# dingwentao/GPU-lossless-compression

Hardware: AMD Instinct MI355X
Metric: encode+decode GB/s (input bytes) per GPU and whole-node; compression ratio parity (higher is better)
Workload: dtype u8; 1 GPU; configs[1]: 4 GiB/GPU Zipf(1.0) bytes (Philox4x32-10, key 0x5eed0002, counter = byte index / 4), 1 MiB blocks, cudppCompress BWT+MTF+Huffman encode; block_bytes=1048576, blocks_per_gpu=4096, batch_rows=2048, batch_rows_asked=2048, output_layout=compact, drain_between_steps=False, parallelism=blocks round-robin over 1 GPU(s), no data-path collective, blocks_left_by_bucket_sorter=0, blocks_left_by_sample_sorter=0

## Files before the change

### gpu-lossless-compression_amd/csrc/mtf.hip

```cpp
#include "glc_device.h"
#include "glc_internal.h"

namespace glc {

constexpr int MTF_WAVES = 4;
constexpr int MTF_INP = 256 + 8;

__global__ __launch_bounds__(MTF_WAVES * 64) void k_mtf_chunk_lists(const uint8_t *__restrict__ in,
                                                                   size_t in_stride, uint32_t n,
                                                                   uint8_t *__restrict__ lists,
                                                                   uint16_t *__restrict__ lens,
                                                                   uint32_t max_chunks, const uint32_t *__restrict__ only)
{
    __shared__ uint32_t s_first[MTF_WAVES][256];
    __shared__ unsigned long long s_bm[MTF_WAVES][64];
    __shared__ uint32_t s_cum[MTF_WAVES][64];
    const uint32_t b = blockIdx.y, l = threadIdx.x & 63;
    if (only && !only[b]) return;
    const uint32_t w = __builtin_amdgcn_readfirstlane(threadIdx.x >> 6);
    const uint32_t chunk = blockIdx.x * MTF_WAVES + w;
    const uint32_t nchunks = (n + MTF_CHUNK - 1) / MTF_CHUNK;
    if (chunk >= nchunks) return;
    const uint32_t lo = chunk * MTF_CHUNK, hi = min(n, lo + MTF_CHUNK), C = hi - lo;
    const uint8_t *src = in + (size_t)b * in_stride;
    uint8_t *L = lists + ((size_t)b * max_chunks + chunk) * 256;
    uint32_t *first = s_first[w];
    for (int i = l; i < 256; i += 64) first[i] = 0xFFFFFFFFu;
    s_bm[w][l] = 0;
    __builtin_amdgcn_wave_barrier();
    if (C == MTF_CHUNK && (reinterpret_cast<uintptr_t>(src + lo) & 15) == 0) {
        uint4 q[4];
#pragma unroll
        for (int g = 0; g < 4; g++)
            q[g] = *reinterpret_cast<const uint4 *>(src + lo + MTF_CHUNK - 1024 * g - 16 * (l + 1));
#pragma unroll
        for (int g = 0; g < 4; g++) {
            const uint32_t d[4] = {q[g].x, q[g].y, q[g].z, q[g].w};
#pragma unroll
            for (int k = 15; k >= 0; k--) {
                const uint32_t sym = (d[k >> 2] >> (8 * (k & 3))) & 0xFFu, o = 1024u * g + 16u * l + 15u - k;
                if (o < first[sym]) atomicMin(&first[sym], o);
            }
        }
    } else {
        for (uint32_t o = l; o < C; o += 64) {
            const uint32_t sym = src[hi - 1 - o];
            if (o < first[sym]) atomicMin(&first[sym], o);
        }
    }
    __builtin_amdgcn_wave_barrier();
    uint32_t f[4];
#pragma unroll
    for (int j = 0; j < 4; j++) {
        f[j] = first[4 * l + j];
        if (f[j] != 0xFFFFFFFFu) atomicOr(&s_bm[w][f[j] >> 6], 1ull << (f[j] & 63));
    }
    __builtin_amdgcn_wave_barrier();
    const uint32_t c = (uint32_t)__popcll(s_bm[w][l]);
    const uint32_t inc = wave_incl_add(c);
    s_cum[w][l] = inc - c;
    __builtin_amdgcn_wave_barrier();
#pragma unroll
    for (int j = 0; j < 4; j++) {
        if (f[j] != 0xFFFFFFFFu) {
            const uint32_t wd = f[j] >> 6, r = f[j] & 63;
            L[s_cum[w][wd] + (uint32_t)__popcll(s_bm[w][wd] & ((1ull << r) - 1ull))] = (uint8_t)(4 * l + j);
        }
    }
    if (l == 0) lens[(size_t)b * max_chunks + chunk] = (uint16_t)__builtin_amdgcn_readlane((int)inc, 63);
}



__device__ __forceinline__ uint32_t mtf_fold(const uint8_t *cur, uint8_t *next, uint8_t *inp, uint32_t p4, uint32_t m,
                                             uint32_t ls, uint32_t l, uint32_t *cur4 = nullptr)
{
    const uint32_t c4 = reinterpret_cast<const uint32_t *>(cur)[l];
    reinterpret_cast<uint32_t *>(inp)[l] = 0;
    __builtin_amdgcn_wave_barrier();
    reinterpret_cast<uint32_t *>(next)[l] = p4;
#pragma unroll
    for (int j = 0; j < 4; j++) inp[4 * l + j < m ? (p4 >> (8 * j)) & 0xFFu : 256u + j] = 1;
    __builtin_amdgcn_wave_barrier();
    if (cur4) *cur4 = c4;
    uint32_t in[4];
#pragma unroll
    for (int j = 0; j < 4; j++) in[j] = inp[(c4 >> (8 * j)) & 0xFFu];
    uint32_t keep[4], cnt = 0;
#pragma unroll
    for (int j = 0; j < 4; j++) { keep[j] = (4 * l + j < ls && !in[j]) ? 1u : 0u; cnt += keep[j]; }
    const uint32_t inc = wave_incl_add(cnt);
    uint32_t pos = m + inc - cnt;
#pragma unroll
    for (int j = 0; j < 4; j++) {
        if (keep[j]) next[pos] = (uint8_t)(c4 >> (8 * j));
        pos += keep[j];
    }
    __builtin_amdgcn_wave_barrier();
    return m + (uint32_t)__builtin_amdgcn_readlane((int)inc, 63);
}

template <int MSC_WAVES>
__global__ __launch_bounds__(MSC_WAVES * 64) void k_mtf_scan_lists(uint8_t *__restrict__ lists,
                                                                  const uint16_t *__restrict__ lens, uint32_t n,
                                                                  uint32_t max_chunks, const uint32_t *__restrict__ only)
{
    constexpr int MSC_GROUP = 256 / MSC_WAVES;
    __shared__ __attribute__((aligned(16))) uint8_t s_state[MSC_WAVES][2][256];
    __shared__ __attribute__((aligned(16))) uint8_t s_inp[MSC_WAVES][MTF_INP];
    __shared__ __attribute__((aligned(16))) uint8_t s_comb[MSC_WAVES][256];
    __shared__ uint32_t s_clen[MSC_WAVES];
    __shared__ __attribute__((aligned(16))) uint8_t s_start[MSC_WAVES + 1][256];
    __shared__ __attribute__((aligned(16))) uint8_t s_carry[256];
    const uint32_t b = blockIdx.x, l = threadIdx.x & 63;
    if (only && !only[b]) return;
    const uint32_t w = __builtin_amdgcn_readfirstlane(threadIdx.x >> 6);
    const uint32_t nchunks = (n + MTF_CHUNK - 1) / MTF_CHUNK;
    uint8_t *LB = lists + (size_t)b * max_chunks * 256;
    const uint16_t *NB = lens + (size_t)b * max_chunks;
    if (w == 0) for (int i = l; i < 256; i += 64) s_carry[i] = (uint8_t)i;
    for (uint32_t r0 = 0; r0 < nchunks; r0 += MSC_WAVES * MSC_GROUP) {
        const uint32_t nch = min(nchunks - r0, (uint32_t)(MSC_WAVES * MSC_GROUP));
        const uint32_t ngroups = (nch + MSC_GROUP - 1) / MSC_GROUP;
        const uint32_t c0 = r0 + w * MSC_GROUP, c1 = min(r0 + nch, c0 + MSC_GROUP);
        uint32_t p4[MSC_GROUP], mm[MSC_GROUP];
#pragma unroll
        for (int k = 0; k < MSC_GROUP; k++) {
            const bool in = c0 + k < c1;
            p4[k] = in ? reinterpret_cast<const uint32_t *>(LB + (size_t)(c0 + k) * 256)[l] : 0u;
            mm[k] = in ? NB[c0 + k] : 0u;
        }
        if (w < ngroups) {
            int cur = 0;
            uint32_t ls = 0;
#pragma unroll
            for (int k = 0; k < MSC_GROUP; k++)
                if (c0 + k < c1) { ls = mtf_fold(s_state[w][cur], s_state[w][cur ^ 1], s_inp[w], p4[k], mm[k], ls, l); cur ^= 1; }
            reinterpret_cast<uint32_t *>(s_comb[w])[l] = reinterpret_cast<const uint32_t *>(s_state[w][cur])[l];
            if (l == 0) s_clen[w] = ls;
        }
        __syncthreads();
        if (w == 0) {
            reinterpret_cast<uint32_t *>(s_start[0])[l] = reinterpret_cast<const uint32_t *>(s_carry)[l];
            uint32_t cp[MSC_WAVES], cl[MSC_WAVES];
#pragma unroll
            for (int g = 0; g < MSC_WAVES; g++) { cp[g] = reinterpret_cast<const uint32_t *>(s_comb[g])[l]; cl[g] = s_clen[g]; }
            __builtin_amdgcn_wave_barrier();
#pragma unroll
            for (int g = 0; g < MSC_WAVES; g++)
                if ((uint32_t)g < ngroups) (void)mtf_fold(s_start[g], s_start[g + 1], s_inp[0], cp[g], cl[g], 256, l);
            reinterpret_cast<uint32_t *>(s_carry)[l] = reinterpret_cast<const uint32_t *>(s_start[ngroups])[l];
        }
        __syncthreads();
        if (w < ngroups) {
            int cur = 0;
            reinterpret_cast<uint32_t *>(s_state[w][0])[l] = reinterpret_cast<const uint32_t *>(s_start[w])[l];
            __builtin_amdgcn_wave_barrier();
#pragma unroll
            for (int k = 0; k < MSC_GROUP; k++) {
                if (c0 + k < c1) {
                    uint32_t st4;
                    if (c0 + k + 1 < c1) { (void)mtf_fold(s_state[w][cur], s_state[w][cur ^ 1], s_inp[w], p4[k], mm[k], 256, l, &st4); cur ^= 1; }
                    else st4 = reinterpret_cast<const uint32_t *>(s_state[w][cur])[l];
                    reinterpret_cast<uint32_t *>(LB + (size_t)(c0 + k) * 256)[l] = st4;
                }
            }
        }
        __syncthreads();
    }
}

constexpr int MTF_ROWS = 4;
constexpr int MTF_NWORDS = 32;
constexpr uint32_t MTF_SEG = 1024;
#ifndef GLC_MTF_QUARTERS_MAX
#define GLC_MTF_QUARTERS_MAX 2048
#endif
constexpr uint32_t MTF_QUARTERS_MAX_CHUNKS = GLC_MTF_QUARTERS_MAX;

__device__ __forceinline__ void mtf_rebase(uint32_t *tab, unsigned long long *bm, uint16_t *cum, uint32_t lr)
{
#pragma unroll 4
    for (int k = 0; k < 16; k++) {
        const uint32_t c = 16u * (uint32_t)k + lr;
        const uint32_t t = tab[c] >> 16, wd = t >> 6;
        const uint32_t kb = cum[wd] + (uint32_t)__popcll(bm[wd] << (63u - (t & 63u)));
        tab[c] = (t - kb) << 16;
    }
    __builtin_amdgcn_wave_barrier();
    bm[2 * lr] = 0; bm[2 * lr + 1] = 0;
    reinterpret_cast<uint32_t *>(cum)[lr] = 0;
    __builtin_amdgcn_wave_barrier();
}

__device__ __forceinline__ uint32_t mtf_slide(uint32_t Pb)
{
    uint32_t G = 0, t0;
#define GLC_SLIDE(K)                                                                                    \
    "v_sub_co_u32_dpp %1, vcc, %2, %2 row_shr:" #K " row_mask:0xf bank_mask:0xf bound_ctrl:1\n\t"            \
    "v_addc_co_u32_e32 %0, vcc, 0, %0, vcc\n\t"
    asm volatile(GLC_SLIDE(1) GLC_SLIDE(2) GLC_SLIDE(3) GLC_SLIDE(4) GLC_SLIDE(5) GLC_SLIDE(6) GLC_SLIDE(7) GLC_SLIDE(8)
                 GLC_SLIDE(9) GLC_SLIDE(10) GLC_SLIDE(11) GLC_SLIDE(12) GLC_SLIDE(13) GLC_SLIDE(14) GLC_SLIDE(15)
                 : "+v"(G), "=&v"(t0) : "v"(Pb) : "vcc");
#undef GLC_SLIDE
    return G;
}

__device__ __forceinline__ void mtf_recount(const unsigned long long *bm, uint16_t *cum, uint32_t lr)
{
    const uint4 v = *reinterpret_cast<const uint4 *>(bm + 2 * lr);
    const uint32_t c0 = (uint32_t)__builtin_popcount(v.x) + (uint32_t)__builtin_popcount(v.y);
    const uint32_t sum = c0 + (uint32_t)__builtin_popcount(v.z) + (uint32_t)__builtin_popcount(v.w);
    uint32_t inc = sum;
    inc += GLC_DPP(inc, 0x111, 0xf);
    inc += GLC_DPP(inc, 0x112, 0xf);
    inc += GLC_DPP(inc, 0x114, 0xf);
    inc += GLC_DPP(inc, 0x118, 0xf);
    const uint32_t r0 = inc - sum;
    reinterpret_cast<uint32_t *>(cum)[lr] = r0 | ((r0 + c0) << 16);
}


#ifndef GLC_MTF_REQ_DIST
#define GLC_MTF_REQ_DIST 1
#endif
constexpr int MTF_REQ = GLC_MTF_REQ_DIST;
#ifndef GLC_MTF_FULL_GROUP
#define GLC_MTF_FULL_GROUP 4
#endif
constexpr int MTF_GROUP = GLC_MTF_FULL_GROUP;
static_assert(MTF_REQ >= 1 && MTF_GROUP % MTF_REQ == 0 && MTF_SEG % (16 * MTF_GROUP) == 0 && MTF_CHUNK % MTF_SEG == 0, "group shape");

template <bool WITH_HIST, bool ZEROS, bool LASTG>
__device__ __forceinline__ void mtf_full_group(const uint8_t *__restrict__ sb, uint8_t *__restrict__ db, uint32_t voff,
                                               uint32_t lbg, uint32_t (&q)[MTF_REQ], uint32_t *tab, unsigned long long *bm,
                                               uint16_t *cum, uint32_t *hist, uint32_t lr, uint32_t row)
{
    const uint32_t mybit = 1u << lr, below = mybit - 1u;
    const uint8_t *sp = sb + voff;
    uint8_t *dp = db + voff;
    uint16_t *killp = reinterpret_cast<uint16_t *>(bm) + ((lbg + 256u) >> 4);
#pragma unroll
    for (int j = 0; j < MTF_GROUP; j++) {
        const uint32_t lb = lbg + 16u * j;
        const uint32_t sym = q[0];
#pragma unroll
        for (int d = 0; d + 1 < MTF_REQ; d++) q[d] = q[d + 1];
        if (!LASTG || j + MTF_REQ < MTF_GROUP) q[MTF_REQ - 1] = sp[16 * (j + MTF_REQ)];
        atomicOr(&tab[sym], mybit);
        __builtin_amdgcn_wave_barrier();
        const uint32_t e = tab[sym];
        const uint32_t before = e & below;
        const bool hasprev = before != 0;
        const uint32_t p = 31u - (uint32_t)__builtin_clz(before | 1u);
        const bool last_in_batch = ((e & 0xFFFFu) >> lr) == 1u;
        uint32_t Pb = hasprev ? lb + p + 257u : (e >> 16) + 1u;
        asm volatile("s_nop 1" : "+v"(Pb));
        const uint32_t T = mtf_slide(Pb) + lr - 15u;
        const uint32_t bitx = Pb - 1u;
        uint32_t o;
        if (hasprev) o = T - (p + 1u);
        else {
            const uint32_t wd = bitx >> 6, r = bitx & 63;
            const uint32_t kb = cum[wd] + (uint32_t)__popcll(bm[wd] << (63u - r));
            o = T + kb + 255u - bitx;
        }
        __builtin_amdgcn_wave_barrier();
        {
            const uint64_t nl = __ballot(!last_in_batch);
            if (lr == 0) killp[j] = (uint16_t)(nl >> (16u * row));
        }
        if (WITH_HIST && ZEROS) {
            const uint64_t zb = __ballot(o == 0);
            const uint32_t zrow = (uint32_t)(zb >> (16u * row)) & 0xFFFFu;
            if (lr == 0 && zrow) atomicAdd(&hist[0], (uint32_t)__builtin_popcount(zrow));
        }
        dp[16 * j] = (uint8_t)o;
        if (WITH_HIST && !(ZEROS && o == 0)) atomicAdd(&hist[o & 127], 1u << ((o >> 3) & 16));
        if (!hasprev) atomicOr(&reinterpret_cast<uint32_t *>(bm)[bitx >> 5], 1u << (bitx & 31));
        if (last_in_batch) tab[sym] = (lb + lr + 256u) << 16;
        __builtin_amdgcn_wave_barrier();
        mtf_recount(bm, cum, lr);
        __builtin_amdgcn_wave_barrier();
    }
}

template <bool WITH_HIST, bool ZEROS>
__device__ __forceinline__ void mtf_encode_full_row(const uint8_t *__restrict__ sb, uint8_t *__restrict__ db, uint32_t lo,
                                                    const uint8_t *__restrict__ list, uint32_t *tab, unsigned long long *bm,
                                                    uint16_t *cum, uint32_t *hist, uint32_t *__restrict__ H, uint32_t lr,
                                                    uint32_t row)
{
    {
        const uint4 lw = reinterpret_cast<const uint4 *>(list)[lr];
        const uint32_t q[4] = {lw.x, lw.y, lw.z, lw.w};
#pragma unroll
        for (int j = 0; j < 16; j++) tab[(q[j >> 2] >> (8 * (j & 3))) & 0xFF] = (255u - (16 * lr + j)) << 16;
        bm[2 * lr] = 0; bm[2 * lr + 1] = 0;
        reinterpret_cast<uint32_t *>(cum)[lr] = 0;
        if (WITH_HIST) for (int i = lr; i < 128; i += 16) hist[i] = 0;
        __builtin_amdgcn_wave_barrier();
    }
    uint32_t voff = lo + lr;
    uint32_t q[MTF_REQ];
#pragma unroll
    for (int d = 0; d < MTF_REQ; d++) q[d] = sb[voff + 16u * d];
    constexpr uint32_t NSEG = MTF_CHUNK / MTF_SEG, NGRP = MTF_SEG / (16 * MTF_GROUP);
    for (uint32_t seg = 0; seg < NSEG; seg++) {
        if (seg) mtf_rebase(tab, bm, cum, lr);
        const uint32_t ng = seg + 1 < NSEG ? NGRP : NGRP - 1;
        for (uint32_t g = 0; g < ng; g++, voff += 16 * MTF_GROUP)
            mtf_full_group<WITH_HIST, ZEROS, false>(sb, db, voff, 16 * MTF_GROUP * g, q, tab, bm, cum, hist, lr, row);
    }
    mtf_full_group<WITH_HIST, ZEROS, true>(sb, db, voff, 16 * MTF_GROUP * (NGRP - 1), q, tab, bm, cum, hist, lr, row);
    if (WITH_HIST) {
        __builtin_amdgcn_wave_barrier();
        if constexpr (SUBHIST_PACKED) for (int i = lr; i < 128; i += 16) H[i] = hist[i];
        else for (int i = lr; i < 256; i += 16) H[i] = (hist[i & 127] >> (16 * (i >> 7))) & 0xFFFFu;
    }
}

template <bool WITH_HIST, bool QUARTERS, bool ZEROS = false, bool FULL = false>
__global__ __launch_bounds__(MTF_WAVES * 64) void k_mtf_encode(const uint8_t *__restrict__ in,
                                                              size_t in_stride, uint32_t n,
                                                              const uint8_t *__restrict__ lists,
                                                              uint32_t max_chunks,
                                                              uint8_t *__restrict__ out, size_t out_stride,
                                                              uint32_t *__restrict__ sub_hist, const uint32_t *__restrict__ only)
{
    __shared__ uint32_t s_hist[WITH_HIST ? MTF_WAVES * MTF_ROWS : 1][128 + 8];
    __shared__ uint32_t s_tab[MTF_WAVES * MTF_ROWS][256 + 8];
    __shared__ __attribute__((aligned(16))) unsigned long long s_bm[MTF_WAVES * MTF_ROWS][MTF_NWORDS + 2];
    __shared__ __attribute__((aligned(16))) uint16_t s_cum[MTF_WAVES * MTF_ROWS][MTF_NWORDS + 8];
    __shared__ __attribute__((aligned(16))) uint8_t s_qstart[QUARTERS ? MTF_WAVES : 1][MTF_ROWS][256];
    __shared__ __attribute__((aligned(16))) uint8_t s_qlist[QUARTERS ? MTF_WAVES : 1][256], s_qinp[QUARTERS ? MTF_WAVES : 1][MTF_INP];
    __shared__ uint32_t s_qfirst[QUARTERS ? MTF_WAVES : 1][256], s_qcum[QUARTERS ? MTF_WAVES : 1][16];
    __shared__ unsigned long long s_qbm[QUARTERS ? MTF_WAVES : 1][16];
    const uint32_t b = blockIdx.y, l = threadIdx.x & 63, lr = l & 15, row = l >> 4;
    if (only && !only[b]) return;
    const uint32_t w = threadIdx.x >> 6, slot = w * MTF_ROWS + row;
    const uint32_t nchunks = (n + MTF_CHUNK - 1) / MTF_CHUNK;
    constexpr uint32_t QLEN = MTF_CHUNK / MTF_ROWS;
    const uint32_t chunk0 = QUARTERS ? blockIdx.x * MTF_WAVES + w : (blockIdx.x * MTF_WAVES + w) * MTF_ROWS;
    if (chunk0 >= nchunks) return;
    const uint32_t chunk = QUARTERS ? chunk0 : chunk0 + row;
    if constexpr (FULL) {
        static_assert(!QUARTERS, "the rows of the FULL form are whole chunks");
        mtf_encode_full_row<WITH_HIST, ZEROS>(in + (size_t)b * in_stride, out + (size_t)b * out_stride, chunk * MTF_CHUNK,
                                              lists + ((size_t)b * max_chunks + chunk) * 256, s_tab[slot], s_bm[slot], s_cum[slot],
                                              s_hist[WITH_HIST ? slot : 0], sub_hist + ((size_t)b * max_chunks + chunk) * SUBHIST_DWORDS, lr, row);
        return;
    }
    const uint32_t Cc0 = min(n, chunk0 * MTF_CHUNK + MTF_CHUNK) - chunk0 * MTF_CHUNK;
    bool live;
    uint32_t lo, C, Cmax;
    if (QUARTERS) {
        live = Cc0 > QLEN * row;
        lo = chunk0 * MTF_CHUNK + (live ? QLEN * row : 0u);
        C = live ? min(Cc0 - QLEN * row, QLEN) : 0u;
        Cmax = min(Cc0, QLEN);
    } else {
        live = chunk < nchunks;
        lo = (live ? chunk : chunk0) * MTF_CHUNK;
        C = live ? min(n, lo + MTF_CHUNK) - lo : 0u;
        Cmax = Cc0;
    }
    const uint8_t *src = in + (size_t)b * in_stride + lo;
    uint8_t *dst = out + (size_t)b * out_stride + lo;
    uint32_t *tab = s_tab[slot];
    unsigned long long *bm = s_bm[slot];
    uint16_t *cum = s_cum[slot];
    uint4 lw;
    if (QUARTERS) {
        uint8_t (*S)[256] = s_qstart[w];
        reinterpret_cast<uint32_t *>(S[0])[l] = reinterpret_cast<const uint32_t *>(lists + ((size_t)b * max_chunks + chunk0) * 256)[l];
        const uint8_t *cbase = in + (size_t)b * in_stride + chunk0 * MTF_CHUNK;
        const bool vec = (reinterpret_cast<uintptr_t>(cbase) & 15) == 0;
        for (uint32_t q = 0; q + 1 < MTF_ROWS && Cc0 > QLEN * (q + 1); q++) {
            uint32_t *first = s_qfirst[w];
            for (int i = l; i < 256; i += 64) first[i] = 0xFFFFFFFFu;
            if (l < 16) s_qbm[w][l] = 0;
            __builtin_amdgcn_wave_barrier();
            const uint8_t *qs = cbase + QLEN * q;
            if (vec) {
                const uint4 v = *reinterpret_cast<const uint4 *>(qs + QLEN - 16 * (l + 1));
                const uint32_t d[4] = {v.x, v.y, v.z, v.w};
#pragma unroll
                for (int k = 15; k >= 0; k--) {
                    const uint32_t sym = (d[k >> 2] >> (8 * (k & 3))) & 0xFFu, o = 16u * l + 15u - k;
                    if (o < first[sym]) atomicMin(&first[sym], o);
                }
            } else {
                for (uint32_t o = l; o < QLEN; o += 64) {
                    const uint32_t sym = qs[QLEN - 1 - o];
                    if (o < first[sym]) atomicMin(&first[sym], o);
                }
            }
            __builtin_amdgcn_wave_barrier();
            uint32_t f[4];
#pragma unroll
            for (int j = 0; j < 4; j++) {
                f[j] = first[4 * l + j];
                if (f[j] != 0xFFFFFFFFu) atomicOr(&s_qbm[w][f[j] >> 6], 1ull << (f[j] & 63));
            }
            __builtin_amdgcn_wave_barrier();
            const uint32_t c = l < 16 ? (uint32_t)__popcll(s_qbm[w][l]) : 0u;
            const uint32_t inc = wave_incl_add(c);
            if (l < 16) s_qcum[w][l] = inc - c;
            __builtin_amdgcn_wave_barrier();
            uint8_t *L = s_qlist[w];
#pragma unroll
            for (int j = 0; j < 4; j++) {
                if (f[j] != 0xFFFFFFFFu) {
                    const uint32_t wd = f[j] >> 6, r = f[j] & 63;
                    L[s_qcum[w][wd] + (uint32_t)__popcll(s_qbm[w][wd] & ((1ull << r) - 1ull))] = (uint8_t)(4 * l + j);
                }
            }
            __builtin_amdgcn_wave_barrier();
            const uint32_t m = (uint32_t)__builtin_amdgcn_readlane((int)inc, 63);
            (void)mtf_fold(S[q], S[q + 1], s_qinp[w], reinterpret_cast<const uint32_t *>(L)[l], m, 256, l);
        }
        __builtin_amdgcn_wave_barrier();
        lw = reinterpret_cast<const uint4 *>(S[live ? row : 0])[lr];
    } else {
        lw = reinterpret_cast<const uint4 *>(lists + ((size_t)b * max_chunks + (live ? chunk : chunk0)) * 256)[lr];
    }
    {
        const uint32_t q[4] = {lw.x, lw.y, lw.z, lw.w};
#pragma unroll
        for (int j = 0; j < 16; j++) tab[(q[j >> 2] >> (8 * (j & 3))) & 0xFF] = (255u - (16 * lr + j)) << 16;
        bm[2 * lr] = 0; bm[2 * lr + 1] = 0;
        reinterpret_cast<uint32_t *>(cum)[lr] = 0;
        if (WITH_HIST) for (int i = lr; i < 128; i += 16) s_hist[slot][i] = 0;
        __builtin_amdgcn_wave_barrier();
    }
    const uint32_t mybit = 1u << lr, below = mybit - 1u;
    uint32_t sym_next = src[lr < C ? lr : 0u];
    for (uint32_t seg0 = 0; seg0 < Cmax; seg0 += MTF_SEG) {
        if (seg0) {
#pragma unroll 4
            for (int k = 0; k < 16; k++) {
                const uint32_t c = 16u * (uint32_t)k + lr;
                const uint32_t t = tab[c] >> 16, wd = t >> 6;
                const uint32_t kb = cum[wd] + (uint32_t)__popcll(bm[wd] << (63u - (t & 63u)));
                tab[c] = (t - kb) << 16;
            }
            __builtin_amdgcn_wave_barrier();
            bm[2 * lr] = 0; bm[2 * lr + 1] = 0;
            reinterpret_cast<uint32_t *>(cum)[lr] = 0;
            __builtin_amdgcn_wave_barrier();
        }
        const uint32_t seg_end = min(Cmax, seg0 + MTF_SEG);
        for (uint32_t base = seg0; base < seg_end; base += 16) {
            const uint32_t i = base + lr, lb = base - seg0;
            const bool valid = i < C;
            const uint32_t sym = sym_next;
            sym_next = src[i + 16 < C ? i + 16 : 0u];
            if (valid) atomicOr(&tab[sym], mybit);
            __builtin_amdgcn_wave_barrier();
            const uint32_t e = tab[sym];
            const uint32_t before = e & below;
            const bool hasprev = before != 0;
            const uint32_t p = 31u - (uint32_t)__builtin_clz(before | 1u);
            const bool last_in_batch = ((e & 0xFFFFu) >> lr) == 1u;
            const uint32_t Pb = hasprev ? lb + p + 257u : (e >> 16) + 1u;
            const uint32_t T = mtf_slide(Pb) + lr - 15u;
            const uint32_t bitx = Pb - 1u;
            uint32_t o;
            if (hasprev) o = T - (p + 1u);
            else {
                const uint32_t wd = bitx >> 6, r = bitx & 63;
                const uint32_t kb = cum[wd] + (uint32_t)__popcll(bm[wd] << (63u - r));
                o = T + kb + 255u - bitx;
            }
            __builtin_amdgcn_wave_barrier();
            {
                const uint64_t nl = __ballot(valid && !last_in_batch);
                const uint32_t half = (row & 2) ? (uint32_t)(nl >> 32) : (uint32_t)nl;
                if (lr == 0) reinterpret_cast<uint16_t *>(bm)[(lb + 256u) >> 4] = (uint16_t)(half >> (16 * (row & 1)));
            }
            if (WITH_HIST && ZEROS) {
                const uint64_t zb = __ballot(valid && o == 0);
                const uint32_t zrow = (uint32_t)(zb >> (16u * row)) & 0xFFFFu;
                if (lr == 0 && zrow) atomicAdd(&s_hist[slot][0], (uint32_t)__builtin_popcount(zrow));
            }
            if (valid) {
                dst[i] = (uint8_t)o;
                if (WITH_HIST && !(ZEROS && o == 0)) atomicAdd(&s_hist[slot][o & 127], 1u << ((o >> 3) & 16));
                if (!hasprev) atomicOr(&reinterpret_cast<uint32_t *>(bm)[bitx >> 5], 1u << (bitx & 31));
                if (last_in_batch) tab[sym] = (lb + lr + 256u) << 16;
            }
            __builtin_amdgcn_wave_barrier();
            mtf_recount(bm, cum, lr);
            __builtin_amdgcn_wave_barrier();
        }
    }
    if (WITH_HIST && QUARTERS) {
        __builtin_amdgcn_wave_barrier();
        uint32_t *H = sub_hist + ((size_t)b * max_chunks + chunk0) * SUBHIST_DWORDS;
        for (int i = l; i < (int)SUBHIST_DWORDS; i += 64) {
            uint32_t c = 0;
#pragma unroll
            for (int r = 0; r < MTF_ROWS; r++)
                c += SUBHIST_PACKED ? s_hist[w * MTF_ROWS + r][i] : (s_hist[w * MTF_ROWS + r][i & 127] >> (16 * (i >> 7))) & 0xFFFFu;
            H[i] = c;
        }
    } else if (WITH_HIST && live) {
        __builtin_amdgcn_wave_barrier();
        uint32_t *H = sub_hist + ((size_t)b * max_chunks + chunk) * SUBHIST_DWORDS;
        if constexpr (SUBHIST_PACKED) for (int i = lr; i < 128; i += 16) H[i] = s_hist[slot][i];
        else for (int i = lr; i < 256; i += 16) H[i] = (s_hist[slot][i & 127] >> (16 * (i >> 7))) & 0xFFFFu;
    }
}

hipError_t mtf_scratch_alloc(MtfScratch &s, uint32_t nmax, uint32_t rows)
{
    s.nmax = nmax; s.rows = rows; s.max_chunks = (nmax + MTF_CHUNK - 1) / MTF_CHUNK;
    size_t a = (size_t)rows * s.max_chunks * 256, c = (size_t)rows * s.max_chunks * sizeof(uint16_t);
    GLC_TRY(hipMalloc((void **)&s.lists, a));
    GLC_TRY(hipMalloc((void **)&s.lens, c));
    s.bytes = a + c;
    return hipSuccess;
}

void mtf_scratch_free(MtfScratch &s)
{
    if (s.lists) (void)hipFree(s.lists);
    if (s.lens) (void)hipFree(s.lens);
    s = MtfScratch();
}

hipError_t mtf_forward(hipStream_t st, const uint8_t *in, size_t in_stride, uint32_t n, uint32_t nblk,
                       uint8_t *out, size_t out_stride, MtfScratch &s, uint32_t *sub_hist, const uint32_t *only, bool skewed)
{
    if (n == 0 || n > s.nmax || nblk == 0 || nblk > s.rows) return hipErrorInvalidValue;
    const uint32_t nchunks = (n + MTF_CHUNK - 1) / MTF_CHUNK;
    dim3 g((nchunks + MTF_WAVES - 1) / MTF_WAVES, nblk), t(MTF_WAVES * 64);
    dim3 ge((nchunks + MTF_WAVES * MTF_ROWS - 1) / (MTF_WAVES * MTF_ROWS), nblk);
    const double units = (double)n * nblk;
    {
        ProfScope ps(s.prof, PROF_MTF_LISTS, st, units);
        hipLaunchKernelGGL(k_mtf_chunk_lists, g, t, 0, st, in, in_stride, n, s.lists, s.lens, s.max_chunks, only);
        if (nblk <= 512)
            hipLaunchKernelGGL(k_mtf_scan_lists<16>, dim3(nblk), dim3(16 * 64), 0, st, s.lists, s.lens, n, s.max_chunks, only);
        else
            hipLaunchKernelGGL(k_mtf_scan_lists<8>, dim3(nblk), dim3(8 * 64), 0, st, s.lists, s.lens, n, s.max_chunks, only);
    }
    {
        ProfScope ps(s.prof, PROF_MTF_ENCODE, st, units);
        const bool quarters = (uint64_t)nchunks * nblk <= MTF_QUARTERS_MAX_CHUNKS;
        if (quarters && sub_hist)
            hipLaunchKernelGGL((k_mtf_encode<true, true>), g, t, 0, st, in, in_stride, n, s.lists, s.max_chunks, out,
                               out_stride, sub_hist, only);
        else if (quarters)
            hipLaunchKernelGGL((k_mtf_encode<false, true>), g, t, 0, st, in, in_stride, n, s.lists, s.max_chunks, out,
                               out_stride, sub_hist, only);
        else if (n % (MTF_ROWS * MTF_CHUNK) == 0 && sub_hist && skewed)
            hipLaunchKernelGGL((k_mtf_encode<true, false, true, true>), ge, t, 0, st, in, in_stride, n, s.lists, s.max_chunks, out,
                               out_stride, sub_hist, only);
        else if (n % (MTF_ROWS * MTF_CHUNK) == 0 && sub_hist)
            hipLaunchKernelGGL((k_mtf_encode<true, false, false, true>), ge, t, 0, st, in, in_stride, n, s.lists, s.max_chunks, out,
                               out_stride, sub_hist, only);
        else if (n % (MTF_ROWS * MTF_CHUNK) == 0)
            hipLaunchKernelGGL((k_mtf_encode<false, false, false, true>), ge, t, 0, st, in, in_stride, n, s.lists, s.max_chunks, out,
                               out_stride, sub_hist, only);
        else if (sub_hist && skewed)
            hipLaunchKernelGGL((k_mtf_encode<true, false, true>), ge, t, 0, st, in, in_stride, n, s.lists, s.max_chunks, out,
                               out_stride, sub_hist, only);
        else if (sub_hist)
            hipLaunchKernelGGL((k_mtf_encode<true, false>), ge, t, 0, st, in, in_stride, n, s.lists, s.max_chunks, out,
                               out_stride, sub_hist, only);
        else
            hipLaunchKernelGGL((k_mtf_encode<false, false>), ge, t, 0, st, in, in_stride, n, s.lists, s.max_chunks, out,
                               out_stride, sub_hist, only);
    }
    return hipGetLastError();
}

}
```

Baseline: 125.0 GB/s.

## Let MTF chunk-list, scan and encode kernels span several chunks per wave

Adds a span parameter K (default 4) so that each wave builds one move-to-front first-occurrence list over K consecutive chunks, with an early exit once all 256 symbols have been seen. The scan and full-row encode kernels work on these longer spans and flush per-chunk sub-histograms at chunk boundaries. The goal is fewer list-building and prefix-scan passes and fewer MTF state reseeds per block. It also raises the default request distance from 1 to 2. In exchange, per-wave work gets longer and parallelism drops, and the new path only runs when the block size divides evenly and the quarters mode is not chosen.

```diff
diff --git a/gpu-lossless-compression_amd/csrc/mtf.hip b/gpu-lossless-compression_amd/csrc/mtf.hip
--- a/gpu-lossless-compression_amd/csrc/mtf.hip
+++ b/gpu-lossless-compression_amd/csrc/mtf.hip
@@ -6,47 +6,77 @@
 constexpr int MTF_WAVES = 4;
 constexpr int MTF_INP = 256 + 8;
 
+__device__ __forceinline__ bool mtf_all_met(const uint32_t *first, uint32_t l)
+{
+    bool all = true;
+#pragma unroll
+    for (int j = 0; j < 4; j++) all = all && first[4 * l + j] != 0xFFFFFFFFu;
+    return __ballot(all) == ~0ull;
+}
+
+template <int K>
 __global__ __launch_bounds__(MTF_WAVES * 64) void k_mtf_chunk_lists(const uint8_t *__restrict__ in,
                                                                    size_t in_stride, uint32_t n,
                                                                    uint8_t *__restrict__ lists,
                                                                    uint16_t *__restrict__ lens,
                                                                    uint32_t max_chunks, const uint32_t *__restrict__ only)
 {
+    constexpr uint32_t SPAN = K * MTF_CHUNK;
     __shared__ uint32_t s_first[MTF_WAVES][256];
-    __shared__ unsigned long long s_bm[MTF_WAVES][64];
-    __shared__ uint32_t s_cum[MTF_WAVES][64];
+    __shared__ unsigned long long s_bm[MTF_WAVES][64 * K];
+    __shared__ uint32_t s_cum[MTF_WAVES][64 * K];
     const uint32_t b = blockIdx.y, l = threadIdx.x & 63;
     if (only && !only[b]) return;
     const uint32_t w = __builtin_amdgcn_readfirstlane(threadIdx.x >> 6);
     const uint32_t chunk = blockIdx.x * MTF_WAVES + w;
-    const uint32_t nchunks = (n + MTF_CHUNK - 1) / MTF_CHUNK;
+    const uint32_t nchunks = (n + SPAN - 1) / SPAN;
     if (chunk >= nchunks) return;
-    const uint32_t lo = chunk * MTF_CHUNK, hi = min(n, lo + MTF_CHUNK), C = hi - lo;
+    const uint32_t lo = chunk * SPAN, hi = min(n, lo + SPAN), C = hi - lo;
     const uint8_t *src = in + (size_t)b * in_stride;
     uint8_t *L = lists + ((size_t)b * max_chunks + chunk) * 256;
     uint32_t *first = s_first[w];
     for (int i = l; i < 256; i += 64) first[i] = 0xFFFFFFFFu;
-    s_bm[w][l] = 0;
-    __builtin_amdgcn_wave_barrier();
-    if (C == MTF_CHUNK && (reinterpret_cast<uintptr_t>(src + lo) & 15) == 0) {
-        uint4 q[4];
-#pragma unroll
-        for (int g = 0; g < 4; g++)
-            q[g] = *reinterpret_cast<const uint4 *>(src + lo + MTF_CHUNK - 1024 * g - 16 * (l + 1));
-#pragma unroll
-        for (int g = 0; g < 4; g++) {
-            const uint32_t d[4] = {q[g].x, q[g].y, q[g].z, q[g].w};
-#pragma unroll
-            for (int k = 15; k >= 0; k--) {
-                const uint32_t sym = (d[k >> 2] >> (8 * (k & 3))) & 0xFFu, o = 1024u * g + 16u * l + 15u - k;
-                if (o < first[sym]) atomicMin(&first[sym], o);
-            }
-        }
-    } else {
+#pragma unroll
+    for (int k = 0; k < K; k++) s_bm[w][K * l + k] = 0;
+    __builtin_amdgcn_wave_barrier();
+    if (C == SPAN && (reinterpret_cast<uintptr_t>(src + lo) & 15) == 0) {
+#pragma unroll
+        for (int c = 0; c < K; c++) {
+            if (K > 1 && c) {
+                __builtin_amdgcn_wave_barrier();
+                if (mtf_all_met(first, l)) break;
+            }
+            uint4 q[4];
+#pragma unroll
+            for (int g = 0; g < 4; g++)
+                q[g] = *reinterpret_cast<const uint4 *>(src + lo + (K - c) * MTF_CHUNK - 1024 * g - 16 * (l + 1));
+#pragma unroll
+            for (int g = 0; g < 4; g++) {
+                const uint32_t d[4] = {q[g].x, q[g].y, q[g].z, q[g].w};
+#pragma unroll
+                for (int k = 15; k >= 0; k--) {
+                    const uint32_t sym = (d[k >> 2] >> (8 * (k & 3))) & 0xFFu, o = 4096u * c + 1024u * g + 16u * l + 15u - k;
+                    if (o < first[sym]) atomicMin(&first[sym], o);
+                }
+            }
+        }
+    } else if constexpr (K == 1) {
         for (uint32_t o = l; o < C; o += 64) {
             const uint32_t sym = src[hi - 1 - o];
             if (o < first[sym]) atomicMin(&first[sym], o);
         }
+    } else {
+        for (uint32_t c0 = 0; c0 < C; c0 += MTF_CHUNK) {
+            if (c0) {
+                __builtin_amdgcn_wave_barrier();
+                if (mtf_all_met(first, l)) break;
+            }
+            const uint32_t c1 = min(C, c0 + MTF_CHUNK);
+            for (uint32_t o = c0 + l; o < c1; o += 64) {
+                const uint32_t sym = src[hi - 1 - o];
+                if (o < first[sym]) atomicMin(&first[sym], o);
+            }
+        }
     }
     __builtin_amdgcn_wave_barrier();
     uint32_t f[4];
@@ -56,9 +86,13 @@
         if (f[j] != 0xFFFFFFFFu) atomicOr(&s_bm[w][f[j] >> 6], 1ull << (f[j] & 63));
     }
     __builtin_amdgcn_wave_barrier();
-    const uint32_t c = (uint32_t)__popcll(s_bm[w][l]);
+    uint32_t ck[K], c = 0;
+#pragma unroll
+    for (int k = 0; k < K; k++) { ck[k] = (uint32_t)__popcll(s_bm[w][K * l + k]); c += ck[k]; }
     const uint32_t inc = wave_incl_add(c);
-    s_cum[w][l] = inc - c;
+    uint32_t below = inc - c;
+#pragma unroll
+    for (int k = 0; k < K; k++) { s_cum[w][K * l + k] = below; below += ck[k]; }
     __builtin_amdgcn_wave_barrier();
 #pragma unroll
     for (int j = 0; j < 4; j++) {
@@ -100,12 +134,11 @@
     return m + (uint32_t)__builtin_amdgcn_readlane((int)inc, 63);
 }
 
-template <int MSC_WAVES>
+template <int MSC_WAVES, int K = 1, int MSC_GROUP = 256 / MSC_WAVES>
 __global__ __launch_bounds__(MSC_WAVES * 64) void k_mtf_scan_lists(uint8_t *__restrict__ lists,
                                                                   const uint16_t *__restrict__ lens, uint32_t n,
                                                                   uint32_t max_chunks, const uint32_t *__restrict__ only)
 {
-    constexpr int MSC_GROUP = 256 / MSC_WAVES;
     __shared__ __attribute__((aligned(16))) uint8_t s_state[MSC_WAVES][2][256];
     __shared__ __attribute__((aligned(16))) uint8_t s_inp[MSC_WAVES][MTF_INP];
     __shared__ __attribute__((aligned(16))) uint8_t s_comb[MSC_WAVES][256];
@@ -115,7 +148,7 @@
     const uint32_t b = blockIdx.x, l = threadIdx.x & 63;
     if (only && !only[b]) return;
     const uint32_t w = __builtin_amdgcn_readfirstlane(threadIdx.x >> 6);
-    const uint32_t nchunks = (n + MTF_CHUNK - 1) / MTF_CHUNK;
+    const uint32_t nchunks = (n + K * MTF_CHUNK - 1) / (K * MTF_CHUNK);
     uint8_t *LB = lists + (size_t)b * max_chunks * 256;
     const uint16_t *NB = lens + (size_t)b * max_chunks;
     if (w == 0) for (int i = l; i < 256; i += 64) s_carry[i] = (uint8_t)i;
@@ -222,14 +255,16 @@
 
 
 #ifndef GLC_MTF_REQ_DIST
-#define GLC_MTF_REQ_DIST 1
+#define GLC_MTF_REQ_DIST 2
 #endif
 constexpr int MTF_REQ = GLC_MTF_REQ_DIST;
-#ifndef GLC_MTF_FULL_GROUP
-#define GLC_MTF_FULL_GROUP 4
+constexpr int MTF_GROUP = 4;
+static_assert(MTF_REQ >= 1 && MTF_GROUP % MTF_REQ == 0 && MTF_SEG % (16 * MTF_GROUP) == 0 && MTF_CHUNK % MTF_SEG == 0, "group shape");
+#ifndef GLC_MTF_SPAN
+#define GLC_MTF_SPAN 4
 #endif
-constexpr int MTF_GROUP = GLC_MTF_FULL_GROUP;
-static_assert(MTF_REQ >= 1 && MTF_GROUP % MTF_REQ == 0 && MTF_SEG % (16 * MTF_GROUP) == 0 && MTF_CHUNK % MTF_SEG == 0, "group shape");
+constexpr int MTF_SPAN = GLC_MTF_SPAN;
+static_assert(MTF_SPAN == 1 || MTF_SPAN == 2 || MTF_SPAN == 4, "spans of 1, 2 or 4 chunks");
 
 template <bool WITH_HIST, bool ZEROS, bool LASTG>
 __device__ __forceinline__ void mtf_full_group(const uint8_t *__restrict__ sb, uint8_t *__restrict__ db, uint32_t voff,
@@ -285,7 +320,7 @@
     }
 }
 
-template <bool WITH_HIST, bool ZEROS>
+template <bool WITH_HIST, bool ZEROS, int K>
 __device__ __forceinline__ void mtf_encode_full_row(const uint8_t *__restrict__ sb, uint8_t *__restrict__ db, uint32_t lo,
                                                     const uint8_t *__restrict__ list, uint32_t *tab, unsigned long long *bm,
                                                     uint16_t *cum, uint32_t *hist, uint32_t *__restrict__ H, uint32_t lr,
@@ -306,21 +341,32 @@
 #pragma unroll
     for (int d = 0; d < MTF_REQ; d++) q[d] = sb[voff + 16u * d];
     constexpr uint32_t NSEG = MTF_CHUNK / MTF_SEG, NGRP = MTF_SEG / (16 * MTF_GROUP);
-    for (uint32_t seg = 0; seg < NSEG; seg++) {
+    for (uint32_t seg = 0; seg < K * NSEG; seg++) {
         if (seg) mtf_rebase(tab, bm, cum, lr);
-        const uint32_t ng = seg + 1 < NSEG ? NGRP : NGRP - 1;
+        if constexpr (K > 1 && WITH_HIST) {
+            if (seg && seg % NSEG == 0) {
+                __builtin_amdgcn_wave_barrier();
+                uint32_t *Hc = H + (size_t)(seg / NSEG - 1) * SUBHIST_DWORDS;
+                if constexpr (SUBHIST_PACKED) for (int i = lr; i < 128; i += 16) Hc[i] = hist[i];
+                else for (int i = lr; i < 256; i += 16) Hc[i] = (hist[i & 127] >> (16 * (i >> 7))) & 0xFFFFu;
+                for (int i = lr; i < 128; i += 16) hist[i] = 0;
+                __builtin_amdgcn_wave_barrier();
+            }
+        }
+        const uint32_t ng = seg + 1 < K * NSEG ? NGRP : NGRP - 1;
         for (uint32_t g = 0; g < ng; g++, voff += 16 * MTF_GROUP)
             mtf_full_group<WITH_HIST, ZEROS, false>(sb, db, voff, 16 * MTF_GROUP * g, q, tab, bm, cum, hist, lr, row);
     }
     mtf_full_group<WITH_HIST, ZEROS, true>(sb, db, voff, 16 * MTF_GROUP * (NGRP - 1), q, tab, bm, cum, hist, lr, row);
     if (WITH_HIST) {
         __builtin_amdgcn_wave_barrier();
-        if constexpr (SUBHIST_PACKED) for (int i = lr; i < 128; i += 16) H[i] = hist[i];
-        else for (int i = lr; i < 256; i += 16) H[i] = (hist[i & 127] >> (16 * (i >> 7))) & 0xFFFFu;
-    }
-}
-
-template <bool WITH_HIST, bool QUARTERS, bool ZEROS = false, bool FULL = false>
+        uint32_t *Hl = H + (size_t)(K - 1) * SUBHIST_DWORDS;
+        if constexpr (SUBHIST_PACKED) for (int i = lr; i < 128; i += 16) Hl[i] = hist[i];
+        else for (int i = lr; i < 256; i += 16) Hl[i] = (hist[i & 127] >> (16 * (i >> 7))) & 0xFFFFu;
+    }
+}
+
+template <bool WITH_HIST, bool QUARTERS, bool ZEROS = false, bool FULL = false, int K = 1>
 __global__ __launch_bounds__(MTF_WAVES * 64) void k_mtf_encode(const uint8_t *__restrict__ in,
                                                               size_t in_stride, uint32_t n,
                                                               const uint8_t *__restrict__ lists,
@@ -342,13 +388,15 @@
     const uint32_t nchunks = (n + MTF_CHUNK - 1) / MTF_CHUNK;
     constexpr uint32_t QLEN = MTF_CHUNK / MTF_ROWS;
     const uint32_t chunk0 = QUARTERS ? blockIdx.x * MTF_WAVES + w : (blockIdx.x * MTF_WAVES + w) * MTF_ROWS;
-    if (chunk0 >= nchunks) return;
+    static_assert(K == 1 || FULL, "only the FULL form has rows of K chunks");
+    if (chunk0 * K >= nchunks) return;
     const uint32_t chunk = QUARTERS ? chunk0 : chunk0 + row;
     if constexpr (FULL) {
         static_assert(!QUARTERS, "the rows of the FULL form are whole chunks");
-        mtf_encode_full_row<WITH_HIST, ZEROS>(in + (size_t)b * in_stride, out + (size_t)b * out_stride, chunk * MTF_CHUNK,
-                                              lists + ((size_t)b * max_chunks + chunk) * 256, s_tab[slot], s_bm[slot], s_cum[slot],
-                                              s_hist[WITH_HIST ? slot : 0], sub_hist + ((size_t)b * max_chunks + chunk) * SUBHIST_DWORDS, lr, row);
+        mtf_encode_full_row<WITH_HIST, ZEROS, K>(in + (size_t)b * in_stride, out + (size_t)b * out_stride, chunk * (K * MTF_CHUNK),
+                                                 lists + ((size_t)b * max_chunks + chunk) * 256, s_tab[slot], s_bm[slot], s_cum[slot],
+                                                 s_hist[WITH_HIST ? slot : 0],
+                                                 sub_hist + ((size_t)b * max_chunks + chunk * K) * SUBHIST_DWORDS, lr, row);
         return;
     }
     const uint32_t Cc0 = min(n, chunk0 * MTF_CHUNK + MTF_CHUNK) - chunk0 * MTF_CHUNK;
@@ -530,6 +578,39 @@
     s = MtfScratch();
 }
 
+template <int K>
+static hipError_t mtf_forward_span(hipStream_t st, const uint8_t *in, size_t in_stride, uint32_t n, uint32_t nblk, uint8_t *out,
+                                   size_t out_stride, MtfScratch &s, uint32_t *sub_hist, const uint32_t *only, bool skewed)
+{
+    if constexpr (K > 1) {
+        const uint32_t nspans = n / (K * MTF_CHUNK);
+        const dim3 t(MTF_WAVES * 64);
+        const double units = (double)n * nblk;
+        {
+            ProfScope ps(s.prof, PROF_MTF_LISTS, st, units);
+            hipLaunchKernelGGL(k_mtf_chunk_lists<K>, dim3((nspans + MTF_WAVES - 1) / MTF_WAVES, nblk), t, 0, st, in, in_stride, n, s.lists,
+                               s.lens, s.max_chunks, only);
+            constexpr int W_FEW = K == 2 ? 16 : 8;
+            if (nblk <= 512)
+                hipLaunchKernelGGL((k_mtf_scan_lists<W_FEW, K, 8>), dim3(nblk), dim3(W_FEW * 64), 0, st, s.lists, s.lens, n, s.max_chunks, only);
+            else
+                hipLaunchKernelGGL((k_mtf_scan_lists<8, K, 32 / K>), dim3(nblk), dim3(8 * 64), 0, st, s.lists, s.lens, n, s.max_chunks, only);
+        }
+        ProfScope ps(s.prof, PROF_MTF_ENCODE, st, units);
+        const dim3 gs((nspans + MTF_WAVES * MTF_ROWS - 1) / (MTF_WAVES * MTF_ROWS), nblk);
+        if (sub_hist && skewed)
+            hipLaunchKernelGGL((k_mtf_encode<true, false, true, true, K>), gs, t, 0, st, in, in_stride, n, s.lists, s.max_chunks, out,
+                               out_stride, sub_hist, only);
+        else if (sub_hist)
+            hipLaunchKernelGGL((k_mtf_encode<true, false, false, true, K>), gs, t, 0, st, in, in_stride, n, s.lists, s.max_chunks, out,
+                               out_stride, sub_hist, only);
+        else
+            hipLaunchKernelGGL((k_mtf_encode<false, false, false, true, K>), gs, t, 0, st, in, in_stride, n, s.lists, s.max_chunks, out,
+                               out_stride, sub_hist, only);
+    }
+    return hipGetLastError();
+}
+
 hipError_t mtf_forward(hipStream_t st, const uint8_t *in, size_t in_stride, uint32_t n, uint32_t nblk,
                        uint8_t *out, size_t out_stride, MtfScratch &s, uint32_t *sub_hist, const uint32_t *only, bool skewed)
 {
@@ -538,9 +619,12 @@
     dim3 g((nchunks + MTF_WAVES - 1) / MTF_WAVES, nblk), t(MTF_WAVES * 64);
     dim3 ge((nchunks + MTF_WAVES * MTF_ROWS - 1) / (MTF_WAVES * MTF_ROWS), nblk);
     const double units = (double)n * nblk;
+    const bool quarters = (uint64_t)nchunks * nblk <= MTF_QUARTERS_MAX_CHUNKS;
+    if (MTF_SPAN > 1 && !quarters && n % (MTF_SPAN * MTF_ROWS * MTF_CHUNK) == 0)
+        return mtf_forward_span<MTF_SPAN>(st, in, in_stride, n, nblk, out, out_stride, s, sub_hist, only, skewed);
     {
         ProfScope ps(s.prof, PROF_MTF_LISTS, st, units);
-        hipLaunchKernelGGL(k_mtf_chunk_lists, g, t, 0, st, in, in_stride, n, s.lists, s.lens, s.max_chunks, only);
+        hipLaunchKernelGGL(k_mtf_chunk_lists<1>, g, t, 0, st, in, in_stride, n, s.lists, s.lens, s.max_chunks, only);
         if (nblk <= 512)
             hipLaunchKernelGGL(k_mtf_scan_lists<16>, dim3(nblk), dim3(16 * 64), 0, st, s.lists, s.lens, n, s.max_chunks, only);
         else
@@ -548,7 +632,6 @@
     }
     {
         ProfScope ps(s.prof, PROF_MTF_ENCODE, st, units);
-        const bool quarters = (uint64_t)nchunks * nblk <= MTF_QUARTERS_MAX_CHUNKS;
         if (quarters && sub_hist)
             hipLaunchKernelGGL((k_mtf_encode<true, true>), g, t, 0, st, in, in_stride, n, s.lists, s.max_chunks, out,
                                out_stride, sub_hist, only);
```

New measurement: 128.5 GB/s (median of 6 runs). 2.8% higher.
